# BraveGroup/DCD

Measured on AMD Instinct MI355X. Metric: images/sec DGDE train step (bs=8, 384x1280), higher is better.
Workload: dtype f32; 1 GPU; DGDE train bs=8 fp32 on 1xMI355X, synthetic KITTI 384x1280 + random kpts_ann (DGDE.yaml, DLA-34+DCNv2, 6 objects/image); global_batch=8, per_gpu_batch=8, input=384x1280, parallelism=dp1, dcn_precision=f32, step_launch=eager, sync_bn=False

## Files before the change

dcd_amd/_lib.py:

```python
import ctypes
import os

_HERE = os.path.dirname(os.path.abspath(__file__))
LIB_PATH = os.path.join(_HERE, "libdcd_hip.so")
_LIB = None

c_void_p, c_int, c_float, c_size_t, c_int64, c_double = (ctypes.c_void_p, ctypes.c_int, ctypes.c_float,
                                                         ctypes.c_size_t, ctypes.c_int64, ctypes.c_double)


class LossRowsArgs(ctypes.Structure):
    _INTS = ("B", "M", "C", "K", "NP", "num_classes", "ch_box2d", "ch_offset", "ch_corner", "ch_corner_unc", "ch_dims",
             "ch_ori_cls", "ch_ori_off", "ch_depth", "ch_depth_unc", "ch_kpts2d", "ch_kpts3d", "trunc_log")
    _FLOATS = ("depth_lo", "depth_hi", "unc_lo", "unc_hi", "depth_weight")
    _POINTERS = ("pois", "reg_mask", "trunc_mask", "find_pcl", "ori_mask", "cls_ids", "centers", "pad_size", "bboxes",
                 "locations", "rotys", "offset_3D", "dimensions", "orientations", "keypoints", "kp_depth_mask", "kpts2d",
                 "kpts3d", "calib_P", "calib", "dim_mean", "kps_pred", "kps_tgt", "kps3d_pred", "kps3d_tgt", "rot", "P_rows",
                 "kmask", "pair_depth", "pair_mask", "cols", "corners_pred", "corners_tgt", "iou3d", "sums", "grad_sums",
                 "grad_pois", "grad_pair", "grad_kps", "grad_kps3d")
    _fields_ = ([(n, c_int) for n in _INTS] + [(n, c_float) for n in _FLOATS] + [("dim_weight", c_float * 3)]
                + [("down_ratio", c_float), ("kd_eps", c_float)] + [(n, c_void_p) for n in _POINTERS])

HEADS_MAX = 16

# ... 68 lines not shown
    "dcd_clip_adamw_workspace_bytes": (c_size_t, [c_int, c_void_p]),
    "dcd_clip_grad_norm_scalars": (c_int, [c_void_p, c_int, c_void_p, c_void_p, c_float, c_void_p, c_size_t, c_void_p]),
    "dcd_adamw_apply": (c_int, [c_void_p, c_int] + [c_void_p] * 7 + [c_double] * 4 + [c_void_p]),
    "dcd_conv1x1_f32": (c_int, [c_void_p, c_void_p, c_int, c_int, c_int, c_void_p, c_void_p, c_void_p, c_int, c_int, c_int64]),
    "dcd_conv1x1_wrw_f32_workspace_bytes": (c_size_t, [c_int, c_int, c_int, c_int64]),
    "dcd_conv1x1_wrw_f32": (c_int, [c_void_p, c_void_p, c_void_p, c_void_p, c_int, c_int, c_int, c_int, c_int64, c_void_p, c_size_t]),
    "dcd_conv3x3_bf16_weights_bytes": (c_size_t, [c_int] * 3),
    "dcd_conv3x3_bf16_transform_weights": (c_int, [c_void_p, c_void_p, c_int, c_int, c_void_p, c_void_p]),
    "dcd_conv3x3_bf16_transform_weights_table": (c_int, [c_void_p, c_void_p, c_int]),
    "dcd_conv3x3_bf16_workspace_bytes": (c_size_t, [c_int] * 5),
    "dcd_conv3x3_bf16_prepared": (c_int, [c_void_p] * 6 + [c_int] * 6 + [c_void_p, c_size_t]),
    "dcd_conv_stem_workspace_bytes": (c_size_t, [c_int] * 3),
    "dcd_conv_stem": (c_int, [c_void_p] * 4 + [c_int] * 7 + [c_void_p, c_size_t]),
    "dcd_conv_stem_wrw_workspace_bytes": (c_size_t, [c_int] * 3),
    "dcd_conv_stem_wrw": (c_int, [c_void_p] * 4 + [c_int] * 6 + [c_void_p, c_size_t]),
    "dcd_context_norm_forward": (c_int, [c_void_p] * 4 + [c_int, c_int, c_float]),
    "dcd_context_norm_backward": (c_int, [c_void_p] * 5 + [c_int, c_int]),
    "dcd_context_norm_relu_add_forward": (c_int, [c_void_p] * 4 + [c_int, c_int, c_float]),
    "dcd_gmw_refine": (c_int, [c_void_p] * 5 + [c_int, c_void_p, c_void_p, c_int, c_int, c_int] + [c_void_p] * 3),
    "dcd_sum_tensors": (c_int, [c_void_p, c_void_p, c_int, c_void_p, c_int64]),
    "dcd_conv3x3_wrw_workspace_bytes": (c_size_t, [c_int] * 5),
    "dcd_conv3x3_wrw": (c_int, [c_void_p] * 4 + [c_int] * 6 + [c_void_p, c_size_t]),
    "dcd_upsample_dw_forward": (c_int, [c_void_p] * 4 + [c_int] * 5),
    "dcd_upsample_dw_forward_add": (c_int, [c_void_p] * 5 + [c_int] * 5),
    "dcd_maxpool2x2_forward": (c_int, [c_void_p, c_void_p, c_void_p, c_int64, c_int, c_int]),
    "dcd_maxpool2x2_backward": (c_int, [c_void_p, c_void_p, c_void_p, c_void_p, c_int64, c_int, c_int]),
    "dcd_upsample_dw_backward": (c_int, [c_void_p] * 6 + [c_int] * 5),
    "dcd_bn_workspace_bytes": (c_size_t, [c_int]),
    "dcd_bn_stats": (c_int, [c_void_p, c_void_p, c_int, c_int, c_int64, c_void_p, c_void_p, c_size_t]),
    "dcd_channel_sums": (c_int, [c_void_p, c_void_p, c_int, c_int, c_int64, c_void_p, c_void_p, c_size_t]),
    "dcd_bn_train_apply": (c_int, [c_void_p] * 6 + [c_double] + [c_void_p] * 3 + [c_float, c_float, c_int] + [c_void_p] * 3
# ... 86 lines not shown
```

dcd_amd/csrc/norm.hip:

```cpp
#include <hip/hip_runtime.h>
#include <stdint.h>
#include <stdlib.h>

#include "../../include/dcd_hip.h"
#include "tuning_env.h"

namespace {

constexpr int BT = 256;
constexpr int CH = 4096;
constexpr int SMAX = 256;

__device__ inline double wave_sum(double v)
{
#pragma unroll
    for (int o = 32; o; o >>= 1) v += __shfl_down(v, o);
    return v;
}

__device__ inline float bn_shift(float bias, float mean, float scale) { return fmaf(-mean, scale, bias); }

__device__ inline void block_sum2(double &a, double &b)
{
    __shared__ double sh[2][BT / 64];
// ... 187 lines not shown
                const float4 r = *reinterpret_cast<const float4 *>(residual + base + i);
                v.x += r.x; v.y += r.y; v.z += r.z; v.w += r.w;
            }
            if (relu) {
                v.x = v.x < 0.f ? 0.f : v.x; v.y = v.y < 0.f ? 0.f : v.y; v.z = v.z < 0.f ? 0.f : v.z; v.w = v.w < 0.f ? 0.f : v.w;
            }
            *reinterpret_cast<float4 *>(y + base + i) = v;
        }
    } else {
        for (long i = lo + threadIdx.x; i < hi; i += BT) {
            float v = fmaf(x[base + i], scale, shift);
            if (residual) v += residual[base + i];
            y[base + i] = (relu && v < 0.f) ? 0.f : v;
        }
    }
}

__global__ __launch_bounds__(BT) void bn_bwd_partial(const float *__restrict__ dy, const float *__restrict__ y,
                                                     const float *__restrict__ x, const float *__restrict__ save_mean,
                                                     Plane g, int S, double *__restrict__ partial,
                                                     const float *__restrict__ invstd = nullptr, float *__restrict__ gw = nullptr,
                                                     float *__restrict__ gb = nullptr, const float *__restrict__ mask_weight = nullptr,
                                                     const float *__restrict__ mask_bias = nullptr, int mask_from_x = 0)
{
    const int c = blockIdx.y, s = blockIdx.x;
    const int P = g.B * g.cpp;
    const bool vec = (g.HW & 3) == 0;
    const float mean = save_mean[c];
    const float msc = mask_from_x ? invstd[c] * (mask_weight ? mask_weight[c] : 1.f) : 0.f;
    const float msh = mask_from_x ? bn_shift(mask_bias ? mask_bias[c] : 0.f, mean, msc) : 0.f;
// ... 573 lines not shown
    if (small_channels(B, C, HW)) {
        hipLaunchKernelGGL(bn_small_bwd, dim3(C), dim3(BT), 0, stream, grad_y, (const float *)nullptr, x, weight, save_mean, save_invstd,
                           grad_x, (float *)nullptr, grad_weight, grad_bias, B, C, (int)(HW / 4), bias, 1);
        return hipGetLastError() == hipSuccess ? DCD_OK : DCD_ERR_LAUNCH;
    }
    const Plane g = make_plane(B, C, HW);
    const int S = slices(g);
    hipLaunchKernelGGL(bn_bwd_partial, dim3(S, C), dim3(BT), 0, stream, grad_y, (const float *)nullptr, x, save_mean, g, S, (double *)ws,
                       save_invstd, (float *)nullptr, (float *)nullptr, weight, bias, 1);
    hipLaunchKernelGGL(bn_bwd_apply, dim3(B * g.cpp, C), dim3(BT), 0, stream, grad_y, (const float *)nullptr, x, weight, save_mean,
                       save_invstd, (const double *)nullptr, (const double *)ws, S, (double)B * (double)HW, grad_x, (float *)nullptr,
                       grad_weight, grad_bias, g, bias, 1);
    return hipGetLastError() == hipSuccess ? DCD_OK : DCD_ERR_LAUNCH;
}

int dcd_bn_at_forward(void *stream_, const float *x, const int64_t *pos, const float *weight, const float *bias,
                      const double *stats, double count, float *running_mean, float *running_var,
                      int64_t *num_batches_tracked, float momentum, float eps, int relu, float *x_at, float *y_at,
                      float *save_mean, float *save_invstd, int B, int C, int64_t HW, int N, void *ws, size_t ws_bytes)
{
    hipStream_t stream = (hipStream_t)stream_;
    (void)hipGetLastError();
    if (!x || !pos || !x_at || !y_at || !save_mean || !save_invstd || bad_shape(B, C, HW) || N <= 0 || !(count >= 1.0))
        return DCD_ERR_BAD_ARG;
    if ((running_mean == nullptr) != (running_var == nullptr)) return DCD_ERR_BAD_ARG;
    const Plane g = make_plane(B, C, HW);
    int S = 0;
    if (!stats) {
        if (!ws || ws_bytes < dcd_bn_workspace_bytes(C)) return DCD_ERR_WORKSPACE;
        S = slices(g);
// ... 61 lines not shown
```

dcd_amd/csrc/stem.hip:

```cpp
#include <hip/hip_runtime.h>
#include <stdint.h>

#include "../../include/dcd_hip.h"
#include "zero_fill.h"
#include "lds_limit.h"

typedef float f32x4 __attribute__((ext_vector_type(4)));

namespace {

constexpr int ST_R = 8;
constexpr int ST_C = 64;
constexpr int ST_RS = 72;
constexpr int ST_DPLANE = ST_R * ST_C + 4;

constexpr int round_odd_mult(int x, int m)
{
    int p = (x + m - 1) / m;
    if ((p & 1) == 0) ++p;
    return p * m;
}

template <int CI, int KS>
struct StemCfg {
// ... 19 lines not shown
    using C = StemCfg<CI, KS>;
    const int e = blockIdx.x * blockDim.x + threadIdx.x;
    if (e >= C::NSTEP * 64) return;
    const int s = e >> 6, l = e & 63;
    const int i = l & 15, k = l >> 4;
    const int j = 4 * s + k;
    float v = 0.f;
    if (j < C::NJ) {
        const int tap = j / CI, c = j - tap * CI;
        const int ty = tap / KS, tx = tap - ty * KS;
        v = mode == 0 ? w[((i * CI + c) * KS + ty) * KS + tx] : w[((c * CI + i) * KS + (KS - 1 - ty)) * KS + (KS - 1 - tx)];
    }
    wp[e] = v;
}

template <int CI, int KS, int PLANE>
__device__ __forceinline__ void stage_window(float *__restrict__ win, const float *__restrict__ xb, int H, int W, int r0, int c0, int tid)
{
    using C = StemCfg<CI, KS>;
    constexpr int Q = ST_RS / 4;
    constexpr int N = CI * C::ROWS * Q;
    constexpr int IT = (N + 255) / 256;
    const int HW = H * W;
    f32x4 v[IT];
    int dst[IT];
#pragma unroll
    for (int i = 0; i < IT; ++i) {
        const int e = tid + 256 * i;
        const int ch = e / (C::ROWS * Q), rem = e - ch * (C::ROWS * Q);
        const int row = rem / Q, q = rem - row * Q;
        const int yy = r0 - C::PAD + row, xx = c0 - 4 + 4 * q;
        v[i] = f32x4{0.f, 0.f, 0.f, 0.f};
        dst[i] = e < N ? ch * PLANE + row * ST_RS + 4 * q : -1;
        if (e < N && yy >= 0 && yy < H && xx >= 0 && xx < W) v[i] = *reinterpret_cast<const f32x4 *>(xb + (size_t)ch * HW + (size_t)yy * W + xx);
    }
#pragma unroll
    for (int i = 0; i < IT; ++i)
        if (dst[i] >= 0) *reinterpret_cast<f32x4 *>(win + dst[i]) = v[i];
}

template <int CI, int KS>
__global__ __launch_bounds__(256) void stem_fwd_f32(const float *__restrict__ x, const float *__restrict__ wp, float *__restrict__ y,
                                                    int H, int W, int tiles_x)
{
    using C = StemCfg<CI, KS>;
    constexpr int PLANE = C::PLANE_F;
    extern __shared__ __attribute__((aligned(16))) float lds[];
    const int tid = threadIdx.x;
    const int lane = tid & 63, wave = tid >> 6;
    const int i16 = lane & 15, k = lane >> 4;
    const int ty = blockIdx.x / tiles_x, tx = blockIdx.x - ty * tiles_x;
    const int b = blockIdx.y;
    const int r0 = ty * ST_R, c0 = tx * ST_C;
    const int HW = H * W;

    float a[C::NSTEP];
#pragma unroll
    for (int s = 0; s < C::NSTEP; ++s) a[s] = wp[s * 64 + lane];

    stage_window<CI, KS, PLANE>(lds, x + (size_t)b * CI * HW, H, W, r0, c0, tid);
    __syncthreads();

#pragma unroll 1
    for (int rr = 0; rr < 2; ++rr) {
        const int row = 2 * wave + rr;
        f32x4 acc[4];
#pragma unroll
        for (int g = 0; g < 4; ++g) acc[g] = f32x4{0.f, 0.f, 0.f, 0.f};
        const float *base = lds + row * ST_RS + i16 + 4 - C::PAD;
#pragma unroll
        for (int s = 0; s < C::NSTEP; ++s) {
            int off;
            if constexpr (CI % 4 == 0) {
                off = joff<CI, KS, PLANE>(4 * s) + k * PLANE;
            } else {
                const int o0 = joff<CI, KS, PLANE>(4 * s), o1 = joff<CI, KS, PLANE>(4 * s + 1);
                const int o2 = joff<CI, KS, PLANE>(4 * s + 2), o3 = joff<CI, KS, PLANE>(4 * s + 3);
                off = k == 0 ? o0 : k == 1 ? o1 : k == 2 ? o2 : o3;
            }
#pragma unroll
            for (int g = 0; g < 4; ++g) acc[g] = __builtin_amdgcn_mfma_f32_16x16x4f32(a[s], base[off + 16 * g], acc[g], 0, 0, 0);
        }
        const int yy = r0 + row;
        if (yy < H) {
#pragma unroll
            for (int g = 0; g < 4; ++g) {
                const int xx = c0 + 16 * g + i16;
                if (xx < W) {
#pragma unroll
                    for (int r = 0; r < 4; ++r) y[((size_t)b * 16 + 4 * k + r) * HW + (size_t)yy * W + xx] = acc[g][r];
                }
            }
        }
    }
}

template <int CI, int KS>
__global__ __launch_bounds__(256) void stem_wrw_f32(const float *__restrict__ x, const float *__restrict__ gy, float *__restrict__ part,
                                                    int B, int H, int W, int tiles_x, int tiles_y)
{
    using C = StemCfg<CI, KS>;
    constexpr int PLANE = C::PLANE_W;
    extern __shared__ __attribute__((aligned(16))) float lds[];
    float *win = lds, *dyt = lds + CI * PLANE;
    const int tid = threadIdx.x;
    const int lane = tid & 63, wave = tid >> 6;
    const int j16 = lane & 15, k = lane >> 4;
    const int HW = H * W;
    const int total = B * tiles_x * tiles_y;

    int boff[C::NB];
#pragma unroll
    for (int nb = 0; nb < C::NB; ++nb) {
        const int j = nb * 16 + j16;
        const int jc = j < C::NJ ? j : 0;
        const int tap = jc / CI, c = jc - tap * CI;
        boff[nb] = c * PLANE + (tap / KS) * ST_RS + tap % KS + k + 4 - C::PAD;
    }
    f32x4 acc[C::NB];
#pragma unroll
    for (int nb = 0; nb < C::NB; ++nb) acc[nb] = f32x4{0.f, 0.f, 0.f, 0.f};

    for (int t = blockIdx.x; t < total; t += gridDim.x) {
        const int b = t / (tiles_x * tiles_y), rem = t - b * (tiles_x * tiles_y);
        const int ty = rem / tiles_x, tx = rem - ty * tiles_x;
        const int r0 = ty * ST_R, c0 = tx * ST_C;
        __syncthreads();
        stage_window<CI, KS, PLANE>(win, x + (size_t)b * CI * HW, H, W, r0, c0, tid);
        const float *gb = gy + (size_t)b * 16 * HW;
        {
            constexpr int ITD = 16 * ST_R * (ST_C / 4) / 256;
            f32x4 v[ITD];
#pragma unroll
            for (int i = 0; i < ITD; ++i) {
                const int e = tid + 256 * i;
                const int o = e / (ST_R * 16), rem2 = e - o * (ST_R * 16);
                const int row = rem2 >> 4, q = rem2 & 15;
                const int yy = r0 + row, xx = c0 + 4 * q;
                v[i] = f32x4{0.f, 0.f, 0.f, 0.f};
                if (yy < H && xx < W) v[i] = *reinterpret_cast<const f32x4 *>(gb + (size_t)o * HW + (size_t)yy * W + xx);
            }
#pragma unroll
            for (int i = 0; i < ITD; ++i) {
                const int e = tid + 256 * i;
                const int o = e / (ST_R * 16), rem2 = e - o * (ST_R * 16);
                *reinterpret_cast<f32x4 *>(dyt + o * ST_DPLANE + (rem2 >> 4) * ST_C + 4 * (rem2 & 15)) = v[i];
            }
        }
        __syncthreads();
#pragma unroll 1
        for (int rr = 0; rr < 2; ++rr) {
            const int row = 2 * wave + rr;
            const float *ap = dyt + j16 * ST_DPLANE + row * ST_C + k;
            const float *bp = win + row * ST_RS;
#pragma unroll 4
            for (int gx = 0; gx < 16; ++gx) {
                const float a = ap[4 * gx];
#pragma unroll
                for (int nb = 0; nb < C::NB; ++nb)
                    acc[nb] = __builtin_amdgcn_mfma_f32_16x16x4f32(a, bp[boff[nb] + 4 * gx], acc[nb], 0, 0, 0);
// ... 9 lines not shown

template <int CI, int KS>
__global__ __launch_bounds__(256) void stem_wrw_reduce(const float *__restrict__ part, int nparts, float *__restrict__ gw)
{
    using C = StemCfg<CI, KS>;
    const int nb = blockIdx.x, e = threadIdx.x;
    const int o = e >> 4, j = nb * 16 + (e & 15);
    float s = 0.f;
    for (int p = blockIdx.y; p < nparts; p += gridDim.y) s += part[((size_t)p * C::NB + nb) * 256 + e];
    if (j < C::NJ) {
        const int tap = j / CI, c = j - tap * CI;
        atomicAdd(gw + (o * CI + c) * C::TAPS + tap, s);
    }
}

template <int CI, int KS>
int launch_fwd(hipStream_t stream, const float *input, const float *weight, float *output, int B, int H, int W, int backward_data,
               float *wp)
{
    using C = StemCfg<CI, KS>;
    static LdsLimit lds_limit;
    const size_t ldsb = (size_t)CI * C::PLANE_F * sizeof(float);
    if (!lds_limit.raise((int)ldsb, stem_fwd_f32<CI, KS>)) return DCD_ERR_LAUNCH;
    hipLaunchKernelGGL((stem_prep_weights<CI, KS>), dim3((C::NSTEP * 64 + 255) / 256), dim3(256), 0, stream, weight, wp, backward_data);
    const int tiles_x = (W + ST_C - 1) / ST_C, tiles_y = (H + ST_R - 1) / ST_R;
    hipLaunchKernelGGL((stem_fwd_f32<CI, KS>), dim3(tiles_x * tiles_y, B), dim3(256), ldsb, stream, input, (const float *)wp, output, H, W,
                       tiles_x);
    return hipGetLastError() == hipSuccess ? DCD_OK : DCD_ERR_LAUNCH;
}

constexpr int ST_WRW_WGS = 512;

template <int CI, int KS>
int launch_wrw(hipStream_t stream, const float *input, const float *grad_output, float *grad_weight, int B, int H, int W, float *part)
{
    using C = StemCfg<CI, KS>;
    static LdsLimit lds_limit;
    const size_t ldsb = (size_t)(CI * C::PLANE_W + 16 * ST_DPLANE) * sizeof(float);
    if (!lds_limit.raise((int)ldsb, stem_wrw_f32<CI, KS>)) return DCD_ERR_LAUNCH;
    const int tiles_x = (W + ST_C - 1) / ST_C, tiles_y = (H + ST_R - 1) / ST_R;
    const int64_t total = (int64_t)B * tiles_x * tiles_y;
    const int nwg = total < ST_WRW_WGS ? (int)total : ST_WRW_WGS;
    if (!dcd_zero_fill(stream, grad_weight, (size_t)16 * C::NJ)) return DCD_ERR_LAUNCH;
    hipLaunchKernelGGL((stem_wrw_f32<CI, KS>), dim3(nwg), dim3(256), ldsb, stream, input, grad_output, part, B, H, W, tiles_x, tiles_y);
    hipLaunchKernelGGL((stem_wrw_reduce<CI, KS>), dim3(C::NB, 32), dim3(256), 0, stream, (const float *)part, nwg * 4, grad_weight);
    return hipGetLastError() == hipSuccess ? DCD_OK : DCD_ERR_LAUNCH;
}

bool stem_shape_ok(int B, int Cin, int H, int W, int Cout, int ksize)
{
    if (B <= 0 || H <= 0 || W <= 0 || (W & 3) || Cout != 16) return false;
    if ((int64_t)B * 16 * H * W >= (1ll << 40)) return false;
    return (Cin == 16 && ksize == 3) || (Cin == 3 && ksize == 7);
}

}

extern "C" {

// ... 24 lines not shown
    if (Cin == 3 && ksize == 7) return (size_t)ST_WRW_WGS * 4 * StemCfg<3, 7>::NB * 256 * sizeof(float);
    return 0;
}

int dcd_conv_stem_wrw(void *stream_, const float *input, const float *grad_output, float *grad_weight, int B, int Cin, int H, int W,
                      int Cout, int ksize, void *workspace, size_t workspace_bytes)
{
    hipStream_t stream = (hipStream_t)stream_;
    (void)hipGetLastError();
    if (!input || !grad_output || !grad_weight || !workspace || !stem_shape_ok(B, Cin, H, W, Cout, ksize)) return DCD_ERR_BAD_ARG;
    if (workspace_bytes < dcd_conv_stem_wrw_workspace_bytes(Cin, Cout, ksize)) return DCD_ERR_WORKSPACE;
    if (Cin == 16) return launch_wrw<16, 3>(stream, input, grad_output, grad_weight, B, H, W, (float *)workspace);
    return launch_wrw<3, 7>(stream, input, grad_output, grad_weight, B, H, W, (float *)workspace);
}

}
```

dcd_amd/model/backbone/dla_dcn.py:

```python
import math
import os

import numpy as np
import torch
from torch import nn

from .DCNv2.dcn_v2 import DCN
from dcd_amd import ops
from dcd_amd.model.layers.norm import BatchNorm2d
from dcd_amd.model.layers.conv import Conv2d, DepthwiseUpsample, MaxPool2x2

BN_MOMENTUM = 0.1
_ROOT_SPLIT = os.environ.get("DCD_ROOT_SPLIT", "1") != "0"


def _bn(c, relu=False):
    return BatchNorm2d(c, momentum=BN_MOMENTUM, fuse_relu=relu)


def _relu_slot():
    return nn.Identity()


class BasicBlock(nn.Module):
# ... 90 lines not shown
        self.level1 = self._make_conv_level(channels[0], channels[1], levels[1], stride=2)
        self.level2 = Tree(levels[2], block, channels[1], channels[2], 2, level_root=False, root_residual=residual_root)
        self.level3 = Tree(levels[3], block, channels[2], channels[3], 2, level_root=True, root_residual=residual_root)
        self.level4 = Tree(levels[4], block, channels[3], channels[4], 2, level_root=True, root_residual=residual_root)
        self.level5 = Tree(levels[5], block, channels[4], channels[5], 2, level_root=True, root_residual=residual_root)

    @staticmethod
    def _make_conv_level(inplanes, planes, convs, stride=1, dilation=1):
        mods = []
        for i in range(convs):
            mods += [Conv2d(inplanes, planes, 3, stride=stride if i == 0 else 1, padding=dilation, bias=False,
                            dilation=dilation), _bn(planes, relu=True), _relu_slot()]
            inplanes = planes
        return nn.Sequential(*mods)

    def forward(self, x):
        maps = []
        x = self.base_layer(x)
        for i in range(6):
            x = getattr(self, "level{}".format(i))(x)
            maps.append(x)
        return maps

    def load_pretrained_model(self, pretrain_path):
        weights = torch.load(pretrain_path, map_location="cpu")
        if isinstance(weights, dict) and "model" in weights:
            prefix = "backbone.bottom_up."
            weights = {k.replace(prefix, ""): v for k, v in weights["model"].items() if prefix in k}
        elif any(k.startswith("fc.") for k in weights):
            n_cls = len(weights[list(weights.keys())[-1]])
            self.fc = nn.Conv2d(self.channels[-1], n_cls, kernel_size=1, stride=1, padding=0, bias=True)
        self.load_state_dict(weights)


# ... 102 lines not shown
```

dcd_amd/ops.py:

```python
import os

import torch

from . import _lib


def _f32c(t):
    if t.dtype != torch.float32:
        t = t.float()
    return t.contiguous()


class _PairsDepth(torch.autograd.Function):
    @staticmethod
    def forward(ctx, kps, kps3d, rot_y, P, kmask, topk, zmin, zmax, normalized, sub_b3):
        _lib.require_cuda(kps, kps3d, rot_y, P)
        L = _lib.lib()
        kps, kps3d, P = _f32c(kps), _f32c(kps3d), _f32c(P)
        rot = _f32c(rot_y).reshape(-1)
        N, K = kps.shape[0], kps.shape[1]
        npairs = K * (K - 1) // 2
        M = topk if topk else npairs
        dev = kps.device
        depth = torch.empty((N, M), dtype=torch.float32, device=dev)
# ... 1294 lines not shown
            L = _lib.lib()
            B, Ci, H, W = x.shape
            Co, k = weight.shape[0], weight.shape[2]
            gw = torch.empty_like(weight)
            n = L.dcd_conv_stem_wrw_workspace_bytes(Ci, Co, k)
            ws = torch.empty(n, dtype=torch.uint8, device=x.device)
            st = L.dcd_conv_stem_wrw(_lib.stream_of(x), x.data_ptr(), gy.data_ptr(), gw.data_ptr(), B, Ci, H, W, Co, k, ws.data_ptr(), n)
            _lib.check(st, "dcd_conv_stem_wrw")
        return gx, gw


def conv_stem(x, weight):
    return _ConvStem.apply(x, weight)


class _ContextNorm(torch.autograd.Function):

    @staticmethod
    def forward(ctx, x, eps):
        _lib.require_cuda(x)
        x = _f32c(x)
        K = x.shape[-1]
        rows = x.numel() // K
        y = torch.empty_like(x)
        inv = torch.empty(rows, dtype=torch.float32, device=x.device)
        _lib.check(_lib.lib().dcd_context_norm_forward(_lib.stream_of(x), x.data_ptr(), y.data_ptr(), inv.data_ptr(), rows, K, float(eps)),
                   "dcd_context_norm_forward")
        ctx.save_for_backward(y, inv)
        return y

# ... 337 lines not shown
```

include/dcd_hip.h:

```cpp
#ifndef DCD_HIP_H
#define DCD_HIP_H

#include <stddef.h>
#include <stdint.h>

#ifdef __cplusplus
extern "C" {
#endif

#define DCD_OK 0
#define DCD_ERR_BAD_ARG 1
#define DCD_ERR_WORKSPACE 2
#define DCD_ERR_LAUNCH 3

const char *dcd_version(void);


#define DCD_PREC_F32 0
#define DCD_PREC_BF16X3 1
#define DCD_PREC_BF16 2

size_t dcd_dcn_v2_workspace_bytes(int B, int Cin, int H, int W, int Cout, int kh, int kw, int sh, int sw,
                                  int ph, int pw, int dh, int dw, int dg);

// ... 220 lines not shown
size_t dcd_conv3x3_s2_f32_wrw_workspace_bytes(int B, int Cin, int H, int W, int Cout);
int dcd_conv3x3_s2_f32_wrw(void *stream, const float *input, const float *grad_output, float *grad_weight, int B, int Cin, int H, int W,
                           int Cout, void *workspace, size_t workspace_bytes);

size_t dcd_conv3x3_wrw_workspace_bytes(int B, int Cin, int H, int W, int Cout);
int dcd_conv3x3_wrw(void *stream, const float *input, const float *grad_output, float *grad_weight, int B, int Cin, int H, int W,
                    int Cout, int precision, void *workspace, size_t workspace_bytes);

size_t dcd_conv_stem_workspace_bytes(int Cin, int Cout, int ksize);
int dcd_conv_stem(void *stream, const float *input, const float *weight, float *output, int B, int Cin, int H, int W, int Cout,
                  int ksize, int backward_data, void *workspace, size_t workspace_bytes);
size_t dcd_conv_stem_wrw_workspace_bytes(int Cin, int Cout, int ksize);
int dcd_conv_stem_wrw(void *stream, const float *input, const float *grad_output, float *grad_weight, int B, int Cin, int H, int W,
                      int Cout, int ksize, void *workspace, size_t workspace_bytes);

int dcd_upsample_dw_forward(void *stream, const float *x, const float *weight, float *y, int B, int C, int H, int W, int f);
int dcd_upsample_dw_forward_add(void *stream, const float *x, const float *weight, const float *skip, float *y, int B, int C, int H,
                                int W, int f);

int dcd_maxpool2x2_forward(void *stream, const float *x, float *y, int64_t planes, int H, int W);
int dcd_maxpool2x2_backward(void *stream, const float *x, const float *grad_y, float *grad_x, int64_t planes, int H, int W);
int dcd_upsample_dw_backward(void *stream, const float *x, const float *weight, const float *grad_y, float *grad_x,
                             float *grad_weight, int B, int C, int H, int W, int f);

int dcd_encode_targets(void *stream, const double *objs, const double *kpts3d, const double *P, const int32_t *img_size,
                       const int32_t *n_obj, int B, int M, int n_extra, int in_w, int in_h, int down_ratio, double filter_trunc,
                       double filter_size, double edge_heatmap_ratio, int num_bin, int n_classes, void *const *outputs,
                       int n_outputs);

int dcd_preprocess_images(void *stream, const uint8_t *src, int64_t src_bytes, const int64_t *images, const float *table, int B,
// ... 67 lines not shown
```

Measured before the change: 215.5 images/s.

## Fuse DLA stem conv+BN+ReLU stages with in-kernel stats and BN-aware weight grads

New measurement: 214.1 images/s. No clear change (-0.6%).

```diff
diff --git a/dcd_amd/_lib.py b/dcd_amd/_lib.py
--- a/dcd_amd/_lib.py
+++ b/dcd_amd/_lib.py
@@ -106,7 +106,12 @@
     "dcd_conv_stem": (c_int, [c_void_p] * 4 + [c_int] * 7 + [c_void_p, c_size_t]),
     "dcd_conv_stem_wrw_workspace_bytes": (c_size_t, [c_int] * 3),
     "dcd_conv_stem_wrw": (c_int, [c_void_p] * 4 + [c_int] * 6 + [c_void_p, c_size_t]),
-    "dcd_context_norm_forward": (c_int, [c_void_p] * 4 + [c_int, c_int, c_float]),
+    "dcd_conv_stem_stat_parts": (c_int64, [c_int] * 3),
+    "dcd_conv_stem_bn": (c_int, [c_void_p] * 4 + [c_int] * 6 + [c_void_p] * 3 + [c_size_t, c_void_p, c_size_t]),
+    "dcd_bn_finalize": (c_int, [c_void_p, c_void_p, c_int64, c_double] + [c_void_p] * 5 + [c_float, c_float] + [c_void_p] * 5 + [c_int]),
+    "dcd_bn_backward_consts_relu_from_x": (c_int, [c_void_p] * 10 + [c_int, c_int, c_int64, c_void_p, c_size_t]),
+    "dcd_conv_stem_wrw_bn": (c_int, [c_void_p] * 4 + [c_int] * 6 + [c_void_p] * 4 + [c_void_p, c_size_t]),
+    "dcd_context_norm_forward":(c_int, [c_void_p] * 4 + [c_int, c_int, c_float]),
     "dcd_context_norm_backward": (c_int, [c_void_p] * 5 + [c_int, c_int]),
     "dcd_context_norm_relu_add_forward": (c_int, [c_void_p] * 4 + [c_int, c_int, c_float]),
     "dcd_gmw_refine": (c_int, [c_void_p] * 5 + [c_int, c_void_p, c_void_p, c_int, c_int, c_int] + [c_void_p] * 3),
diff --git a/dcd_amd/csrc/norm.hip b/dcd_amd/csrc/norm.hip
--- a/dcd_amd/csrc/norm.hip
+++ b/dcd_amd/csrc/norm.hip
@@ -225,6 +225,71 @@
             y[base + i] = (relu && v < 0.f) ? 0.f : v;
         }
     }
+}
+
+__global__ __launch_bounds__(64) void bn_finalize(const double *__restrict__ partial, int S, double count, const float *__restrict__ weight,
+                                                  const float *__restrict__ bias, float *__restrict__ running_mean,
+                                                  float *__restrict__ running_var, long long *__restrict__ num_batches_tracked,
+                                                  float momentum, float eps, float *__restrict__ scale_out, float *__restrict__ shift_out,
+                                                  float *__restrict__ save_mean, float *__restrict__ save_invstd, double *__restrict__ sums)
+{
+    constexpr int U = 16;
+    const int c = blockIdx.x;
+    const double2 *p = reinterpret_cast<const double2 *>(partial) + (long)c * S;
+    double s0 = 0.0, s1 = 0.0;
+    for (int s = threadIdx.x; s < S; s += 64 * U) {
+        double2 v[U];
+#pragma unroll
+        for (int u = 0; u < U; ++u) v[u] = s + 64 * u < S ? p[s + 64 * u] : make_double2(0.0, 0.0);
+#pragma unroll
+        for (int u = 0; u < U; ++u) { s0 += v[u].x; s1 += v[u].y; }
+    }
+    s0 = wave_sum(s0);
+    s1 = wave_sum(s1);
+    if (threadIdx.x != 0) return;
+    const double m = s0 / count;
+    double var = s1 / count - m * m;
+    var = var < 0.0 ? 0.0 : var;
+    const float mean = (float)m;
+    const float invstd = (float)(1.0 / sqrt(var + (double)eps));
+    save_mean[c] = mean;
+    save_invstd[c] = invstd;
+    if (running_mean) {
+        const double unbiased = count > 1.0 ? var * (count / (count - 1.0)) : var;
+        running_mean[c] = (1.f - momentum) * running_mean[c] + momentum * mean;
+        running_var[c] = (1.f - momentum) * running_var[c] + momentum * (float)unbiased;
+    }
+    if (num_batches_tracked && c == 0) *num_batches_tracked += 1;
+    const float scale = invstd * (weight ? weight[c] : 1.f);
+    scale_out[c] = scale;
+    shift_out[c] = bn_shift(bias ? bias[c] : 0.f, mean, scale);
+    if (sums) { sums[2 * c] = s0; sums[2 * c + 1] = s1; }
+}
+
+__global__ __launch_bounds__(64) void bn_bwd_finalize(const double *__restrict__ partial, int S, double count, const float *__restrict__ weight,
+                                                      const float *__restrict__ bias, const float *__restrict__ save_mean,
+                                                      const float *__restrict__ save_invstd, float *__restrict__ dweight,
+                                                      float *__restrict__ dbias, float *__restrict__ consts, int C)
+{
+    const int c = blockIdx.x;
+    double s0 = 0.0, s1 = 0.0;
+    for (int s = threadIdx.x; s < S; s += 64) {
+        s0 += partial[((long)c * S + s) * 2 + 0];
+        s1 += partial[((long)c * S + s) * 2 + 1];
+    }
+    s0 = wave_sum(s0);
+    s1 = wave_sum(s1);
+    if (threadIdx.x != 0) return;
+    const float mean = save_mean[c], invstd = save_invstd[c];
+    const float msc = invstd * (weight ? weight[c] : 1.f);
+    const float msh = bn_shift(bias ? bias[c] : 0.f, mean, msc);
+    if (dweight) dweight[c] = (float)(s1 * (double)invstd);
+    if (dbias) dbias[c] = (float)s0;
+    consts[0 * C + c] = mean;
+    consts[1 * C + c] = msc;
+    consts[2 * C + c] = msh;
+    consts[3 * C + c] = (float)(s0 / count);
+    consts[4 * C + c] = (float)(s1 / count * (double)invstd * (double)invstd);
 }
 
 __global__ __launch_bounds__(BT) void bn_bwd_partial(const float *__restrict__ dy, const float *__restrict__ y,
@@ -828,6 +893,36 @@
     return hipGetLastError() == hipSuccess ? DCD_OK : DCD_ERR_LAUNCH;
 }
 
+int dcd_bn_finalize(void *stream_, const double *stat_part, int64_t parts, double count, const float *weight, const float *bias,
+                    float *running_mean, float *running_var, int64_t *num_batches_tracked, float momentum, float eps, float *scale,
+                    float *shift, float *save_mean, float *save_invstd, double *sums, int C)
+{
+    (void)hipGetLastError();
+    if (!stat_part || !scale || !shift || !save_mean || !save_invstd || C <= 0 || C > 65535 || parts <= 0 || parts > (1ll << 30) || !(count >= 1.0))
+        return DCD_ERR_BAD_ARG;
+    if ((running_mean == nullptr) != (running_var == nullptr)) return DCD_ERR_BAD_ARG;
+    hipLaunchKernelGGL(bn_finalize, dim3(C), dim3(64), 0, (hipStream_t)stream_, stat_part, (int)parts, count, weight, bias, running_mean,
+                       running_var, (long long *)num_batches_tracked, momentum, eps, scale, shift, save_mean, save_invstd, sums);
+    return hipGetLastError() == hipSuccess ? DCD_OK : DCD_ERR_LAUNCH;
+}
+
+int dcd_bn_backward_consts_relu_from_x(void *stream_, const float *grad_y, const float *x, const float *weight, const float *bias,
+                                       const float *save_mean, const float *save_invstd, float *grad_weight, float *grad_bias,
+                                       float *consts, int B, int C, int64_t HW, void *ws, size_t ws_bytes)
+{
+    hipStream_t stream = (hipStream_t)stream_;
+    (void)hipGetLastError();
+    if (!grad_y || !x || !save_mean || !save_invstd || !consts || bad_shape(B, C, HW)) return DCD_ERR_BAD_ARG;
+    if (!ws || ws_bytes < dcd_bn_workspace_bytes(C)) return DCD_ERR_WORKSPACE;
+    const Plane g = make_plane(B, C, HW);
+    const int S = slices(g);
+    hipLaunchKernelGGL(bn_bwd_partial, dim3(S, C), dim3(BT), 0, stream, grad_y, (const float *)nullptr, x, save_mean, g, S, (double *)ws,
+                       save_invstd, (float *)nullptr, (float *)nullptr, weight, bias, 1);
+    hipLaunchKernelGGL(bn_bwd_finalize, dim3(C), dim3(64), 0, stream, (const double *)ws, S, (double)B * (double)HW, weight, bias, save_mean,
+                       save_invstd, grad_weight, grad_bias, consts, C);
+    return hipGetLastError() == hipSuccess ? DCD_OK : DCD_ERR_LAUNCH;
+}
+
 int dcd_bn_at_forward(void *stream_, const float *x, const int64_t *pos, const float *weight, const float *bias,
                       const double *stats, double count, float *running_mean, float *running_var,
                       int64_t *num_batches_tracked, float momentum, float eps, int relu, float *x_at, float *y_at,
diff --git a/dcd_amd/csrc/stem.hip b/dcd_amd/csrc/stem.hip
--- a/dcd_amd/csrc/stem.hip
+++ b/dcd_amd/csrc/stem.hip
@@ -57,8 +57,9 @@
     wp[e] = v;
 }
 
-template <int CI, int KS, int PLANE>
-__device__ __forceinline__ void stage_window(float *__restrict__ win, const float *__restrict__ xb, int H, int W, int r0, int c0, int tid)
+template <int CI, int KS, int PLANE, bool AFF = false>
+__device__ __forceinline__ void stage_window(float *__restrict__ win, const float *__restrict__ xb, int H, int W, int r0, int c0, int tid,
+                                             const float *__restrict__ in_scale = nullptr, const float *__restrict__ in_shift = nullptr)
 {
     using C = StemCfg<CI, KS>;
     constexpr int Q = ST_RS / 4;
@@ -67,6 +68,7 @@
     const int HW = H * W;
     f32x4 v[IT];
     int dst[IT];
+    float sc[AFF ? IT : 1], sh[AFF ? IT : 1];
 #pragma unroll
     for (int i = 0; i < IT; ++i) {
         const int e = tid + 256 * i;
@@ -75,16 +77,29 @@
         const int yy = r0 - C::PAD + row, xx = c0 - 4 + 4 * q;
         v[i] = f32x4{0.f, 0.f, 0.f, 0.f};
         dst[i] = e < N ? ch * PLANE + row * ST_RS + 4 * q : -1;
-        if (e < N && yy >= 0 && yy < H && xx >= 0 && xx < W) v[i] = *reinterpret_cast<const f32x4 *>(xb + (size_t)ch * HW + (size_t)yy * W + xx);
-    }
-#pragma unroll
-    for (int i = 0; i < IT; ++i)
+        if constexpr (AFF) sc[i] = sh[i] = 0.f;
+        if (e < N && yy >= 0 && yy < H && xx >= 0 && xx < W) {
+            v[i] = *reinterpret_cast<const f32x4 *>(xb + (size_t)ch * HW + (size_t)yy * W + xx);
+            if constexpr (AFF) { sc[i] = in_scale[ch]; sh[i] = in_shift[ch]; }
+        }
+    }
+#pragma unroll
+    for (int i = 0; i < IT; ++i) {
+        if constexpr (AFF) {
+#pragma unroll
+            for (int r = 0; r < 4; ++r) {
+                const float t = fmaf(v[i][r], sc[i], sh[i]);
+                v[i][r] = t < 0.f ? 0.f : t;
+            }
+        }
         if (dst[i] >= 0) *reinterpret_cast<f32x4 *>(win + dst[i]) = v[i];
-}
-
-template <int CI, int KS>
+    }
+}
+
+template <int CI, int KS, bool AFF = false, bool STAT = false>
 __global__ __launch_bounds__(256) void stem_fwd_f32(const float *__restrict__ x, const float *__restrict__ wp, float *__restrict__ y,
-                                                    int H, int W, int tiles_x)
+                                                    int H, int W, int tiles_x, const float *__restrict__ in_scale = nullptr,
+                                                    const float *__restrict__ in_shift = nullptr, double *__restrict__ stat_part = nullptr)
 {
     using C = StemCfg<CI, KS>;
     constexpr int PLANE = C::PLANE_F;
@@ -101,9 +116,10 @@
 #pragma unroll
     for (int s = 0; s < C::NSTEP; ++s) a[s] = wp[s * 64 + lane];
 
-    stage_window<CI, KS, PLANE>(lds, x + (size_t)b * CI * HW, H, W, r0, c0, tid);
+    stage_window<CI, KS, PLANE, AFF>(lds, x + (size_t)b * CI * HW, H, W, r0, c0, tid, in_scale, in_shift);
     __syncthreads();
 
+    float fs[4] = {0.f, 0.f, 0.f, 0.f}, fq[4] = {0.f, 0.f, 0.f, 0.f};
 #pragma unroll 1
     for (int rr = 0; rr < 2; ++rr) {
         const int row = 2 * wave + rr;
@@ -132,15 +148,53 @@
                 if (xx < W) {
 #pragma unroll
                     for (int r = 0; r < 4; ++r) y[((size_t)b * 16 + 4 * k + r) * HW + (size_t)yy * W + xx] = acc[g][r];
+                    if constexpr (STAT) {
+#pragma unroll
+                        for (int r = 0; r < 4; ++r) {
+                            fs[r] += acc[g][r];
+                            fq[r] = fmaf(acc[g][r], acc[g][r], fq[r]);
+                        }
+                    }
                 }
             }
         }
     }
-}
-
-template <int CI, int KS>
+    if constexpr (STAT) {
+        double ds[4], dq[4];
+#pragma unroll
+        for (int r = 0; r < 4; ++r) {
+            ds[r] = (double)fs[r];
+            dq[r] = (double)fq[r];
+#pragma unroll
+            for (int o = 8; o; o >>= 1) {
+                ds[r] += __shfl_xor(ds[r], o);
+                dq[r] += __shfl_xor(dq[r], o);
+            }
+        }
+        __syncthreads();
+        double *ws = reinterpret_cast<double *>(lds);
+        if (i16 == 0) {
+#pragma unroll
+            for (int r = 0; r < 4; ++r) {
+                ws[(wave * 16 + 4 * k + r) * 2 + 0] = ds[r];
+                ws[(wave * 16 + 4 * k + r) * 2 + 1] = dq[r];
+            }
+        }
+        __syncthreads();
+        if (tid < 32) {
+            const int c = tid >> 1, j = tid & 1;
+            const double v = ((ws[(0 * 16 + c) * 2 + j] + ws[(1 * 16 + c) * 2 + j]) + ws[(2 * 16 + c) * 2 + j]) + ws[(3 * 16 + c) * 2 + j];
+            const size_t nwg = (size_t)gridDim.x * gridDim.y, wg = (size_t)blockIdx.y * gridDim.x + blockIdx.x;
+            stat_part[((size_t)c * nwg + wg) * 2 + j] = v;
+        }
+    }
+}
+
+template <int CI, int KS, int MODE = 0>
 __global__ __launch_bounds__(256) void stem_wrw_f32(const float *__restrict__ x, const float *__restrict__ gy, float *__restrict__ part,
-                                                    int B, int H, int W, int tiles_x, int tiles_y)
+                                                    int B, int H, int W, int tiles_x, int tiles_y, const float *__restrict__ in_scale = nullptr,
+                                                    const float *__restrict__ in_shift = nullptr, const float *__restrict__ bn_x = nullptr,
+                                                    const float *__restrict__ bn_consts = nullptr)
 {
     using C = StemCfg<CI, KS>;
     constexpr int PLANE = C::PLANE_W;
@@ -151,6 +205,10 @@
     const int j16 = lane & 15, k = lane >> 4;
     const int HW = H * W;
     const int total = B * tiles_x * tiles_y;
+    __shared__ float cs[MODE == 2 ? 80 : 1];
+    if constexpr (MODE == 2) {
+        if (tid < 80) cs[tid] = bn_consts[tid];
+    }
 
     int boff[C::NB];
 #pragma unroll
@@ -169,11 +227,12 @@
         const int ty = rem / tiles_x, tx = rem - ty * tiles_x;
         const int r0 = ty * ST_R, c0 = tx * ST_C;
         __syncthreads();
-        stage_window<CI, KS, PLANE>(win, x + (size_t)b * CI * HW, H, W, r0, c0, tid);
+        stage_window<CI, KS, PLANE, MODE == 1>(win, x + (size_t)b * CI * HW, H, W, r0, c0, tid, in_scale, in_shift);
         const float *gb = gy + (size_t)b * 16 * HW;
         {
             constexpr int ITD = 16 * ST_R * (ST_C / 4) / 256;
             f32x4 v[ITD];
+            f32x4 u[MODE == 2 ? ITD : 1];
 #pragma unroll
             for (int i = 0; i < ITD; ++i) {
                 const int e = tid + 256 * i;
@@ -181,12 +240,27 @@
                 const int row = rem2 >> 4, q = rem2 & 15;
                 const int yy = r0 + row, xx = c0 + 4 * q;
                 v[i] = f32x4{0.f, 0.f, 0.f, 0.f};
-                if (yy < H && xx < W) v[i] = *reinterpret_cast<const f32x4 *>(gb + (size_t)o * HW + (size_t)yy * W + xx);
+                if constexpr (MODE == 2) u[i] = f32x4{0.f, 0.f, 0.f, 0.f};
+                if (yy < H && xx < W) {
+                    v[i] = *reinterpret_cast<const f32x4 *>(gb + (size_t)o * HW + (size_t)yy * W + xx);
+                    if constexpr (MODE == 2) u[i] = *reinterpret_cast<const f32x4 *>(bn_x + ((size_t)b * 16 + o) * HW + (size_t)yy * W + xx);
+                }
             }
 #pragma unroll
             for (int i = 0; i < ITD; ++i) {
                 const int e = tid + 256 * i;
                 const int o = e / (ST_R * 16), rem2 = e - o * (ST_R * 16);
+                if constexpr (MODE == 2) {
+                    const int yy = r0 + (rem2 >> 4), xx = c0 + 4 * (rem2 & 15);
+                    if (yy < H && xx < W) {
+                        const float mean = cs[o], k1 = cs[16 + o], msh = cs[32 + o], a = cs[48 + o], bq = cs[64 + o];
+#pragma unroll
+                        for (int r = 0; r < 4; ++r) {
+                            const float d = fmaf(u[i][r], k1, msh) <= 0.f ? 0.f : v[i][r];
+                            v[i][r] = (d - a - (u[i][r] - mean) * bq) * k1;
+                        }
+                    }
+                }
                 *reinterpret_cast<f32x4 *>(dyt + o * ST_DPLANE + (rem2 >> 4) * ST_C + 4 * (rem2 & 15)) = v[i];
             }
         }
@@ -226,35 +300,37 @@
     }
 }
 
-template <int CI, int KS>
+template <int CI, int KS, bool AFF = false, bool STAT = false>
 int launch_fwd(hipStream_t stream, const float *input, const float *weight, float *output, int B, int H, int W, int backward_data,
-               float *wp)
+               float *wp, const float *in_scale = nullptr, const float *in_shift = nullptr, double *stat_part = nullptr)
 {
     using C = StemCfg<CI, KS>;
     static LdsLimit lds_limit;
     const size_t ldsb = (size_t)CI * C::PLANE_F * sizeof(float);
-    if (!lds_limit.raise((int)ldsb, stem_fwd_f32<CI, KS>)) return DCD_ERR_LAUNCH;
+    if (!lds_limit.raise((int)ldsb, stem_fwd_f32<CI, KS, AFF, STAT>)) return DCD_ERR_LAUNCH;
     hipLaunchKernelGGL((stem_prep_weights<CI, KS>), dim3((C::NSTEP * 64 + 255) / 256), dim3(256), 0, stream, weight, wp, backward_data);
     const int tiles_x = (W + ST_C - 1) / ST_C, tiles_y = (H + ST_R - 1) / ST_R;
-    hipLaunchKernelGGL((stem_fwd_f32<CI, KS>), dim3(tiles_x * tiles_y, B), dim3(256), ldsb, stream, input, (const float *)wp, output, H, W,
-                       tiles_x);
+    hipLaunchKernelGGL((stem_fwd_f32<CI, KS, AFF, STAT>), dim3(tiles_x * tiles_y, B), dim3(256), ldsb, stream, input, (const float *)wp,
+                       output, H, W, tiles_x, in_scale, in_shift, stat_part);
     return hipGetLastError() == hipSuccess ? DCD_OK : DCD_ERR_LAUNCH;
 }
 
 constexpr int ST_WRW_WGS = 512;
 
-template <int CI, int KS>
-int launch_wrw(hipStream_t stream, const float *input, const float *grad_output, float *grad_weight, int B, int H, int W, float *part)
+template <int CI, int KS, int MODE = 0>
+int launch_wrw(hipStream_t stream, const float *input, const float *grad_output, float *grad_weight, int B, int H, int W, float *part,
+               const float *in_scale = nullptr, const float *in_shift = nullptr, const float *bn_x = nullptr, const float *bn_consts = nullptr)
 {
     using C = StemCfg<CI, KS>;
     static LdsLimit lds_limit;
     const size_t ldsb = (size_t)(CI * C::PLANE_W + 16 * ST_DPLANE) * sizeof(float);
-    if (!lds_limit.raise((int)ldsb, stem_wrw_f32<CI, KS>)) return DCD_ERR_LAUNCH;
+    if (!lds_limit.raise((int)ldsb, stem_wrw_f32<CI, KS, MODE>)) return DCD_ERR_LAUNCH;
     const int tiles_x = (W + ST_C - 1) / ST_C, tiles_y = (H + ST_R - 1) / ST_R;
     const int64_t total = (int64_t)B * tiles_x * tiles_y;
     const int nwg = total < ST_WRW_WGS ? (int)total : ST_WRW_WGS;
     if (!dcd_zero_fill(stream, grad_weight, (size_t)16 * C::NJ)) return DCD_ERR_LAUNCH;
-    hipLaunchKernelGGL((stem_wrw_f32<CI, KS>), dim3(nwg), dim3(256), ldsb, stream, input, grad_output, part, B, H, W, tiles_x, tiles_y);
+    hipLaunchKernelGGL((stem_wrw_f32<CI, KS, MODE>), dim3(nwg), dim3(256), ldsb, stream, input, grad_output, part, B, H, W, tiles_x, tiles_y,
+                       in_scale, in_shift, bn_x, bn_consts);
     hipLaunchKernelGGL((stem_wrw_reduce<CI, KS>), dim3(C::NB, 32), dim3(256), 0, stream, (const float *)part, nwg * 4, grad_weight);
     return hipGetLastError() == hipSuccess ? DCD_OK : DCD_ERR_LAUNCH;
 }
@@ -309,4 +385,40 @@
     return launch_wrw<3, 7>(stream, input, grad_output, grad_weight, B, H, W, (float *)workspace);
 }
 
-}
+int64_t dcd_conv_stem_stat_parts(int B, int H, int W)
+{
+    if (B <= 0 || H <= 0 || W <= 0) return 0;
+    return (int64_t)B * ((W + ST_C - 1) / ST_C) * ((H + ST_R - 1) / ST_R);
+}
+
+int dcd_conv_stem_bn(void *stream_, const float *input, const float *weight, float *output, int B, int Cin, int H, int W, int Cout,
+                     int ksize, const float *in_scale, const float *in_shift, double *stat_part, size_t stat_bytes, void *workspace,
+                     size_t workspace_bytes)
+{
+    hipStream_t stream = (hipStream_t)stream_;
+    (void)hipGetLastError();
+    if (!input || !weight || !output || !workspace || !stat_part || !stem_shape_ok(B, Cin, H, W, Cout, ksize)) return DCD_ERR_BAD_ARG;
+    if ((in_scale == nullptr) != (in_shift == nullptr) || (in_scale && Cin != 16)) return DCD_ERR_BAD_ARG;
+    if (workspace_bytes < dcd_conv_stem_workspace_bytes(Cin, Cout, ksize)) return DCD_ERR_WORKSPACE;
+    if (stat_bytes < (size_t)dcd_conv_stem_stat_parts(B, H, W) * 16 * 2 * sizeof(double)) return DCD_ERR_WORKSPACE;
+    if (Cin == 16 && in_scale)
+        return launch_fwd<16, 3, true, true>(stream, input, weight, output, B, H, W, 0, (float *)workspace, in_scale, in_shift, stat_part);
+    if (Cin == 16) return launch_fwd<16, 3, false, true>(stream, input, weight, output, B, H, W, 0, (float *)workspace, nullptr, nullptr, stat_part);
+    return launch_fwd<3, 7, false, true>(stream, input, weight, output, B, H, W, 0, (float *)workspace, nullptr, nullptr, stat_part);
+}
+
+int dcd_conv_stem_wrw_bn(void *stream_, const float *input, const float *grad_output, float *grad_weight, int B, int Cin, int H, int W,
+                         int Cout, int ksize, const float *in_scale, const float *in_shift, const float *bn_x, const float *bn_consts,
+                         void *workspace, size_t workspace_bytes)
+{
+    hipStream_t stream = (hipStream_t)stream_;
+    (void)hipGetLastError();
+    if (!input || !grad_output || !grad_weight || !workspace || !stem_shape_ok(B, Cin, H, W, Cout, ksize)) return DCD_ERR_BAD_ARG;
+    const bool aff = in_scale && in_shift && !bn_x && !bn_consts, bwd = bn_x && bn_consts && !in_scale && !in_shift;
+    if (!((aff && Cin == 16) || (bwd && Cin == 3))) return DCD_ERR_BAD_ARG;
+    if (workspace_bytes < dcd_conv_stem_wrw_workspace_bytes(Cin, Cout, ksize)) return DCD_ERR_WORKSPACE;
+    if (aff) return launch_wrw<16, 3, 1>(stream, input, grad_output, grad_weight, B, H, W, (float *)workspace, in_scale, in_shift);
+    return launch_wrw<3, 7, 2>(stream, input, grad_output, grad_weight, B, H, W, (float *)workspace, nullptr, nullptr, bn_x, bn_consts);
+}
+
+}
diff --git a/dcd_amd/model/backbone/dla_dcn.py b/dcd_amd/model/backbone/dla_dcn.py
--- a/dcd_amd/model/backbone/dla_dcn.py
+++ b/dcd_amd/model/backbone/dla_dcn.py
@@ -4,10 +4,12 @@
 import numpy as np
 import torch
 from torch import nn
+from torch.nn.modules import module as _module_hooks
 
 from .DCNv2.dcn_v2 import DCN
 from dcd_amd import ops
 from dcd_amd.model.layers.norm import BatchNorm2d
+from dcd_amd.model.layers import conv as conv_layers
 from dcd_amd.model.layers.conv import Conv2d, DepthwiseUpsample, MaxPool2x2
 
 BN_MOMENTUM = 0.1
@@ -128,10 +130,35 @@
             inplanes = planes
         return nn.Sequential(*mods)
 
+    def _stem_fused_ok(self, x):
+        seqs = (self.base_layer, self.level0)
+        if not (self.training and len(self.level0) == 3 and conv_layers._ENABLED and conv_layers._STEM):
+            return False
+        for seq in seqs:
+            conv, bn, slot = seq[0], seq[1], seq[2]
+            if not (type(conv) is Conv2d and type(bn) is BatchNorm2d and type(slot) is nn.Identity and conv.bias is None
+                    and conv.stride == (1, 1) and conv.dilation == (1, 1) and conv.groups == 1 and conv.padding_mode == "zeros"
+                    and conv.padding == (conv.kernel_size[0] // 2, conv.kernel_size[1] // 2)
+                    and bn.training and bn.fuse_relu and bn.sync_group is None and bn.weight is not None and bn.bias is not None
+                    and bn.momentum is not None):
+                return False
+            for m in (seq, conv, bn, slot):
+                if m._forward_hooks or m._forward_pre_hooks or m._backward_hooks or m._backward_pre_hooks:
+                    return False
+        if _module_hooks._global_forward_hooks or _module_hooks._global_forward_pre_hooks or _module_hooks._global_backward_hooks \
+                or _module_hooks._global_backward_pre_hooks:
+            return False
+        return ops.stem_fused_supported(x, self.base_layer[0].weight, self.level0[0].weight)
+
+    def stem(self, x):
+        if self._stem_fused_ok(x):
+            return ops.stem_fused(x, self.base_layer[0].weight, self.base_layer[1], self.level0[0].weight, self.level0[1])
+        return self.level0(self.base_layer(x))
+
     def forward(self, x):
-        maps = []
-        x = self.base_layer(x)
-        for i in range(6):
+        x = self.stem(x)
+        maps = [x]
+        for i in range(1, 6):
             x = getattr(self, "level{}".format(i))(x)
             maps.append(x)
         return maps
diff --git a/dcd_amd/ops.py b/dcd_amd/ops.py
--- a/dcd_amd/ops.py
+++ b/dcd_amd/ops.py
@@ -1332,6 +1332,107 @@
     return _ConvStem.apply(x, weight)
 
 
+_STEM_FUSE = os.environ.get("DCD_STEM_FUSE", "1") != "0"
+
+
+def stem_fused_supported(x, w0, w1):
+    return (_STEM_FUSE and x.is_cuda and x.dtype == torch.float32 and x.dim() == 4 and not x.requires_grad
+            and tuple(w0.shape) == (16, 3, 7, 7) and tuple(w1.shape) == (16, 16, 3, 3) and w0.dtype == w1.dtype == torch.float32
+            and x.shape[1] == 3 and x.shape[0] > 0 and x.shape[2] > 0 and x.shape[3] > 0 and x.shape[3] % 4 == 0
+            and x.shape[0] * 16 * x.shape[2] * x.shape[3] < (1 << 40))
+
+
+def _stem_conv_stats(inp, weight, in_scale, in_shift):
+    L = _lib.lib()
+    B, Ci, H, W = inp.shape
+    k = weight.shape[2]
+    out = torch.empty((B, 16, H, W), dtype=torch.float32, device=inp.device)
+    parts = L.dcd_conv_stem_stat_parts(B, H, W)
+    stat = torch.empty((16, parts, 2), dtype=torch.float64, device=inp.device)
+    n = L.dcd_conv_stem_workspace_bytes(Ci, 16, k)
+    ws = torch.empty(n, dtype=torch.uint8, device=inp.device)
+    _lib.check(L.dcd_conv_stem_bn(_lib.stream_of(inp), inp.data_ptr(), weight.data_ptr(), out.data_ptr(), B, Ci, H, W, 16, k,
+                                  _lib.ptr(in_scale), _lib.ptr(in_shift), stat.data_ptr(), stat.numel() * 8, ws.data_ptr(), n),
+               "dcd_conv_stem_bn")
+    return out, stat, parts
+
+
+def _stem_bn_finalize(x, stat, parts, weight, bias, running_mean, running_var, nbt, momentum, eps, want_sums):
+    dev = x.device
+    vec = torch.empty((4, 16), dtype=torch.float32, device=dev)
+    sums = torch.empty((16, 2), dtype=torch.float64, device=dev) if want_sums else None
+    count = float(x.shape[0] * x.shape[2] * x.shape[3])
+    _lib.check(_lib.lib().dcd_bn_finalize(_lib.stream_of(x), stat.data_ptr(), parts, count, weight.data_ptr(), bias.data_ptr(),
+                                          _lib.ptr(running_mean), _lib.ptr(running_var), _lib.ptr(nbt), float(momentum), float(eps),
+                                          vec[0].data_ptr(), vec[1].data_ptr(), vec[2].data_ptr(), vec[3].data_ptr(), _lib.ptr(sums), 16),
+               "dcd_bn_finalize")
+    return vec, sums, count
+
+
+class _StemFused(torch.autograd.Function):
+    @staticmethod
+    def forward(ctx, x, w0, g0, b0, rm0, rv0, nbt0, mom0, eps0, w1, g1, b1, rm1, rv1, nbt1, mom1, eps1):
+        _lib.require_cuda(x, w0, g0, b0, w1, g1, b1)
+        L = _lib.lib()
+        x, w0, w1 = _f32c(x), _f32c(w0), _f32c(w1)
+        g0, b0, g1, b1 = _f32c(g0), _f32c(b0), _f32c(g1), _f32c(b1)
+        B, _, H, W = x.shape
+        st = _lib.stream_of(x)
+        x0, stat0, parts = _stem_conv_stats(x, w0, None, None)
+        v0, _, _ = _stem_bn_finalize(x0, stat0, parts, g0, b0, rm0, rv0, nbt0, mom0, eps0, False)
+        x1, stat1, parts = _stem_conv_stats(x0, w1, v0[0], v0[1])
+        v1, sums1, count = _stem_bn_finalize(x1, stat1, parts, g1, b1, rm1, rv1, nbt1, mom1, eps1, True)
+        y1 = torch.empty_like(x1)
+        _lib.check(L.dcd_bn_train_apply(st, x1.data_ptr(), None, g1.data_ptr(), b1.data_ptr(), sums1.data_ptr(), count, None, None, None,
+                                        0.0, float(eps1), 1, y1.data_ptr(), v1[2].data_ptr(), v1[3].data_ptr(), B, 16, H * W),
+                   "dcd_bn_train_apply")
+        ctx.save_for_backward(x, w0, x0, g0, b0, v0, w1, x1, g1, b1, v1)
+        return y1
+
+    @staticmethod
+    @torch.autograd.function.once_differentiable
+    def backward(ctx, gy):
+        x, w0, x0, g0, b0, v0, w1, x1, g1, b1, v1 = ctx.saved_tensors
+        L = _lib.lib()
+        gy = _f32c(gy)
+        B, _, H, W = x.shape
+        HW = H * W
+        dev, st = x.device, _lib.stream_of(x)
+        ws = _bn_ws(16, dev)
+        gx1 = torch.empty_like(x1)
+        gg1 = torch.empty(16, dtype=torch.float32, device=dev)
+        gb1 = torch.empty(16, dtype=torch.float32, device=dev)
+        _lib.check(L.dcd_bn_backward_relu_from_x(st, gy.data_ptr(), x1.data_ptr(), g1.data_ptr(), b1.data_ptr(), v1[2].data_ptr(),
+                                                 v1[3].data_ptr(), gx1.data_ptr(), gg1.data_ptr(), gb1.data_ptr(), B, 16, HW,
+                                                 ws.data_ptr(), ws.numel()), "dcd_bn_backward_relu_from_x")
+        del gy
+        gy0 = _conv_stem_call(gx1, w1, True)
+        gw1 = torch.empty_like(w1)
+        n = L.dcd_conv_stem_wrw_workspace_bytes(16, 16, 3)
+        wws = torch.empty(n, dtype=torch.uint8, device=dev)
+        _lib.check(L.dcd_conv_stem_wrw_bn(st, x0.data_ptr(), gx1.data_ptr(), gw1.data_ptr(), B, 16, H, W, 16, 3, v0[0].data_ptr(),
+                                          v0[1].data_ptr(), None, None, wws.data_ptr(), n), "dcd_conv_stem_wrw_bn")
+        del gx1
+        gg0 = torch.empty(16, dtype=torch.float32, device=dev)
+        gb0 = torch.empty(16, dtype=torch.float32, device=dev)
+        consts = torch.empty((5, 16), dtype=torch.float32, device=dev)
+        _lib.check(L.dcd_bn_backward_consts_relu_from_x(st, gy0.data_ptr(), x0.data_ptr(), g0.data_ptr(), b0.data_ptr(), v0[2].data_ptr(),
+                                                        v0[3].data_ptr(), gg0.data_ptr(), gb0.data_ptr(), consts.data_ptr(), B, 16, HW,
+                                                        ws.data_ptr(), ws.numel()), "dcd_bn_backward_consts_relu_from_x")
+        gw0 = torch.empty_like(w0)
+        n = L.dcd_conv_stem_wrw_workspace_bytes(3, 16, 7)
+        wws = torch.empty(n, dtype=torch.uint8, device=dev)
+        _lib.check(L.dcd_conv_stem_wrw_bn(st, x.data_ptr(), gy0.data_ptr(), gw0.data_ptr(), B, 3, H, W, 16, 7, None, None, x0.data_ptr(),
+                                          consts.data_ptr(), wws.data_ptr(), n), "dcd_conv_stem_wrw_bn")
+        return (None, gw0, gg0, gb0, None, None, None, None, None, gw1, gg1, gb1, None, None, None, None, None)
+
+
+def stem_fused(x, w0, bn0, w1, bn1):
+    return _StemFused.apply(x, w0, bn0.weight, bn0.bias, bn0.running_mean, bn0.running_var, bn0.num_batches_tracked, bn0.momentum,
+                            bn0.eps, w1, bn1.weight, bn1.bias, bn1.running_mean, bn1.running_var, bn1.num_batches_tracked,
+                            bn1.momentum, bn1.eps)
+
+
 class _ContextNorm(torch.autograd.Function):
 
     @staticmethod
diff --git a/include/dcd_hip.h b/include/dcd_hip.h
--- a/include/dcd_hip.h
+++ b/include/dcd_hip.h
@@ -258,6 +258,20 @@
 int dcd_conv_stem_wrw(void *stream, const float *input, const float *grad_output, float *grad_weight, int B, int Cin, int H, int W,
                       int Cout, int ksize, void *workspace, size_t workspace_bytes);
 
+int64_t dcd_conv_stem_stat_parts(int B, int H, int W);
+int dcd_conv_stem_bn(void *stream, const float *input, const float *weight, float *output, int B, int Cin, int H, int W, int Cout,
+                     int ksize, const float *in_scale, const float *in_shift, double *stat_part, size_t stat_bytes, void *workspace,
+                     size_t workspace_bytes);
+int dcd_bn_finalize(void *stream, const double *stat_part, int64_t parts, double count, const float *weight, const float *bias,
+                    float *running_mean, float *running_var, int64_t *num_batches_tracked, float momentum, float eps, float *scale,
+                    float *shift, float *save_mean, float *save_invstd, double *sums, int C);
+int dcd_bn_backward_consts_relu_from_x(void *stream, const float *grad_y, const float *x, const float *weight, const float *bias,
+                                       const float *save_mean, const float *save_invstd, float *grad_weight, float *grad_bias,
+                                       float *consts, int B, int C, int64_t HW, void *workspace, size_t workspace_bytes);
+int dcd_conv_stem_wrw_bn(void *stream, const float *input, const float *grad_output, float *grad_weight, int B, int Cin, int H, int W,
+                         int Cout, int ksize, const float *in_scale, const float *in_shift, const float *bn_x, const float *bn_consts,
+                         void *workspace, size_t workspace_bytes);
+
 int dcd_upsample_dw_forward(void *stream, const float *x, const float *weight, float *y, int B, int C, int H, int W, int f);
 int dcd_upsample_dw_forward_add(void *stream, const float *x, const float *weight, const float *skip, float *y, int B, int C, int H,
                                 int W, int f);
```
